# Gaukler/PlainRenderer

Hardware: AMD Instinct MI355X
Metric: frames/sec full GI+shade+post @4K; %HBM roofline; 1/2/4/8-GPU scaling (higher is better)
Workload: dtype f32

## Files before the change

### plainrenderer_amd/csrc/backend.cpp

```cpp
#include "backend.h"
#include "kernels_fast/pcf_taps.h"

#include <dlfcn.h>
#include <deque>
#include <algorithm>
#include <chrono>
#include <mutex>
#include <cstdlib>
#include <atomic>
#include <set>
#include <thread>
#include <unordered_map>
#include <unordered_set>
#include <cmath>
#include <cstring>
#include <map>
#include <memory>

#include "../../include/plr.h"

namespace plr {

struct ShaderEntry { std::string name; LaunchFn fn = nullptr; LaunchFn fast = nullptr; };
static bool shaderReadsBindless(const std::string& shader) {
// ... 211 lines not shown
    std::vector<FillOrder> fills;
    std::vector<uint8_t> fillData;
    static constexpr int kPinnedSlots = 3;
    struct PinnedSlot { void* host = nullptr; size_t size = 0; hipEvent_t free = nullptr; bool busy = false, eventPending = false; uint64_t serial = 0; } pinnedSlots[kPinnedSlots];
    uint64_t fillSerial = 0;
    uint32_t* edgeSignal = nullptr;
    uint32_t* edgeCounter = nullptr;
    uint32_t edgeSerial = 0;
    uint32_t pinnedNext = 0;
    uint32_t globalUbo = PLR_INVALID_INDEX;
    uint32_t layoutUbufs = 0, layoutSamplers = 0, layoutSampled = 0;
    bool layoutSet = false;
    ImgView* bindlessDev = nullptr;
    std::vector<ImgView> bindlessHost;
    uint32_t bindlessCapacity = 0;
    bool bindlessDirty = true;
    uint64_t allocated = 0;
    bool passTiming = false;
    int mathMode = PLR_MATH_FAST;
    std::vector<hipEvent_t> passEvents;
    struct Segment { size_t firstEvent; const char* name; };
    std::vector<Segment> segments;
    size_t eventsUsed = 0;
    const char* currentPassName = nullptr;
    bool timingNow = false;
    std::vector<plr_renderpass_time> lastTimings;
    std::set<std::string> callbackNames;
    size_t timedExecutions = 0;
    hipEvent_t frameStart = nullptr, frameEnd = nullptr;
    bool frameRecorded = false;
    bool frameTimeAsked = false;
    float lastFrameGpuMs = 0.f;
    float lastCpuMs = 0.f;
    static constexpr int kSideStreams = 3;
    hipStream_t sideStreams[kSideStreams] = {nullptr, nullptr, nullptr};
    std::vector<hipEvent_t> orderEvents;
    size_t orderEventsUsed = 0;
    bool overlap = false;
    int activeSideStreams = 1;
    hipStream_t curStream = nullptr;
    uint32_t lastOverlapped = 0;
    uint32_t* debugSig = nullptr;
    size_t debugSigWords = 0;
    int fusion = 2;
    GlobalUbo globalShadow{};
    bool globalShadowValid = false;
    uint32_t lastFused = 0;
    uint32_t lastGeneral = 0;
    std::string lastGeneralNames;
    uint64_t frameSerial = 0;
    hipStream_t tailStream = nullptr;
    hipEvent_t tailDone = nullptr, tailStart = nullptr;
    uint8_t* pendingFillSlot = nullptr;
    hipEvent_t pendingFillEvent = nullptr;

    hipStream_t earlyStream = nullptr;
    int earlyParts = 0;
    uint32_t lastEarly = 0;
    uint64_t mainOps = 0, tailStartOps = ~0ull;
    bool tailStartCoversLate = false, lateLaunchedThisFrame = false;
    std::vector<const void*> lastFillDsts;
    std::vector<EarlyPlan> earlyPlans;

    std::vector<Access> tailPending;
    bool asyncTail = true;
    bool fusionReorder = true;
    uint32_t lastAsync = 0;
    void* globalCopies[2] = {nullptr, nullptr};
    uint32_t globalCopyIndex = 0;
    std::set<std::string> fusedNames;
    std::unordered_map<const void*, uint64_t> contentVersion;
    std::unordered_set<const void*> externallyWritable;
};

static thread_local Backend* g = nullptr;
static thread_local std::string g_err;

static std::mutex g_exactSetMutex;
static bool g_exactSetTried = false;
static void* g_exactSetHandle = nullptr;
static std::string g_exactSetError;
static int ensureExactSet() {
    std::lock_guard<std::mutex> lock(g_exactSetMutex);
    if (!g_exactSetTried) {
        g_exactSetTried = true;
        Dl_info info{};
        std::string path;
        if (dladdr((const void*)&ensureExactSet, &info) && info.dli_fname) {
            path = info.dli_fname;
            const size_t slash = path.find_last_of('/');
            const size_t name = slash == std::string::npos ? 0 : slash + 1;
            if (path.compare(name, 6, "libplr") == 0) path.insert(name + 6, "_exact");
            else path.clear();
        }
        if (path.empty()) g_exactSetError = "cannot locate libplr.so to find libplr_exact.so next to it";
        else {
            g_exactSetHandle = dlopen(path.c_str(), RTLD_NOW | RTLD_LOCAL);
            if (!g_exactSetHandle) g_exactSetError = "the PLR_MATH_EXACT kernel set is a separate library and it did not load (" + path + "): " + (dlerror() ? dlerror() : "?") +
                                                     " - build it with plainrenderer_amd/build.py";
        }
    }
    if (!g_exactSetHandle) { g_err = g_exactSetError; return PLR_ERR_UNSUPPORTED; }
    return PLR_OK;
}

static std::string shaderBaseName(const std::string& path) {
// ... 222 lines not shown
        right = std::min(std::max(right, 0), (int)blocksX - left);
    }
    if (top + bottom > totalRows) return false;
    if (top + bottom + left + right == 0) return false;
    edgeTop = top; edgeBottom = bottom; total = totalRows;
    edgeLeft = left; edgeRight = right;
    edgeBlocks = (uint32_t)(top + bottom) * blocksX + (uint32_t)(left + right) * (uint32_t)(totalRows - top - bottom);
    edgeCounter = c.edgeCounter; edgeSignal = c.edgeSignal; edgeValue = c.edgeValue;
    if (edgeBlocks == 0) { edgeTop = edgeBottom = edgeLeft = edgeRight = 0; total = 0; return false; }
    static const bool orderOnly = std::getenv("PLR_EDGE_ORDER_ONLY") && std::atoi(std::getenv("PLR_EDGE_ORDER_ONLY")) != 0;
    if (orderOnly) { edgeBlocks = 0; return false; }
    c.edgeSignalHonoured = true;
    return true;
}

void countFusedExecutions(uint32_t n) { if (g) g->lastFused += n; }

}

using namespace plr;

extern "C" {

const char* plr_last_error(void) { return g_err.c_str(); }

int plr_setup(int device_ordinal, uint32_t width, uint32_t height) {
    if (g && g_adopted) { g = nullptr; g_adopted = false; }
    if (g) return setErr(PLR_ERR_INVALID_ARGUMENT, "plr_setup called twice; call plr_shutdown first");
    int count = 0;
    hipError_t e = hipGetDeviceCount(&count);
    if (e != hipSuccess || count == 0)
        return setErr(PLR_ERR_HIP, std::string("no HIP device available: ") + hipGetErrorString(e) + " (this backend has no CPU fallback)");
    if (device_ordinal < 0 || device_ordinal >= count) return setErr(PLR_ERR_INVALID_ARGUMENT, "device ordinal out of range");
    HIP_TRY(hipSetDevice(device_ordinal));
    g_ownedOnce = true;
    g = new Backend();
    {
        Backend* none = nullptr;
        g_first.compare_exchange_strong(none, g);
    }
    g->device = device_ordinal;
    int leastPriority = 0, greatestPriority = 0;
    if (hipDeviceGetStreamPriorityRange(&leastPriority, &greatestPriority) != hipSuccess) { (void)hipGetLastError(); leastPriority = greatestPriority = 0; }
    static const int mainPriority = std::getenv("PLR_MAIN_PRIORITY") ? std::atoi(std::getenv("PLR_MAIN_PRIORITY")) : 0;
    static const int earlyPriority = std::getenv("PLR_EARLY_PRIORITY") ? std::atoi(std::getenv("PLR_EARLY_PRIORITY")) : 0;
    if (mainPriority) HIP_TRY(hipStreamCreateWithPriority(&g->stream, hipStreamNonBlocking, greatestPriority));
    else HIP_TRY(hipStreamCreateWithFlags(&g->stream, hipStreamNonBlocking));
    HIP_TRY(hipEventCreate(&g->frameStart));
    HIP_TRY(hipEventCreate(&g->frameEnd));
    for (auto& slot : g->pinnedSlots) HIP_TRY(hipEventCreateWithFlags(&slot.free, hipEventDisableTiming));
    for (auto& st : g->sideStreams) HIP_TRY(hipStreamCreateWithFlags(&st, hipStreamNonBlocking));
    HIP_TRY(hipStreamCreateWithFlags(&g->tailStream, hipStreamNonBlocking));
    HIP_TRY(hipEventCreateWithFlags(&g->tailDone, hipEventDisableTiming));
    HIP_TRY(hipEventCreateWithFlags(&g->tailStart, hipEventDisableTiming));
    if (earlyPriority) HIP_TRY(hipStreamCreateWithPriority(&g->earlyStream, hipStreamNonBlocking, leastPriority));
    else HIP_TRY(hipStreamCreateWithFlags(&g->earlyStream, hipStreamNonBlocking));
    if (std::getenv("PLR_STREAM_DEBUG")) fprintf(stderr, "[plr streams] priority range least %d greatest %d; main %s, early %s\n", leastPriority, greatestPriority, mainPriority ? "greatest" : "default", earlyPriority ? "least" : "default");
    if (const char* ep = std::getenv("PLR_EARLY_PARTS")) g->earlyParts = std::min(std::max(std::atoi(ep), 0), 2);
    int canWaitValue = 0;
    if (hipDeviceGetAttribute(&canWaitValue, hipDeviceAttributeCanUseStreamWaitValue, device_ordinal) != hipSuccess) { (void)hipGetLastError(); canWaitValue = 0; }
    if (canWaitValue && hipExtMallocWithFlags((void**)&g->edgeSignal, 8, hipMallocSignalMemory) == hipSuccess && hipMalloc((void**)&g->edgeCounter, 4096) == hipSuccess) {
        HIP_TRY(hipMemset(g->edgeSignal, 0, 8));
        HIP_TRY(hipMemset(g->edgeCounter, 0, 4096));
    } else {
        (void)hipGetLastError();
        if (g->edgeSignal) hipFree(g->edgeSignal);
        g->edgeSignal = nullptr; g->edgeCounter = nullptr;
    }
    if (const char* es = std::getenv("PLR_EDGE_SIGNAL")) if (std::atoi(es) == 0 && g->edgeSignal) { hipFree(g->edgeSignal); hipFree(g->edgeCounter); g->edgeSignal = g->edgeCounter = nullptr; }
    if (const char* at = std::getenv("PLR_ASYNC_TAIL")) g->asyncTail = std::atoi(at) != 0;
    if (const char* ov = std::getenv("PLR_STREAM_OVERLAP")) g->overlap = std::atoi(ov) != 0;
    if (const char* pf = std::getenv("PLR_PASS_FUSION")) g->fusion = std::min(std::max(std::atoi(pf), 0), 2);
    if (const char* ns = std::getenv("PLR_SIDE_STREAMS")) g->activeSideStreams = std::min(std::max(std::atoi(ns), 1), (int)Backend::kSideStreams);
    return plr_recreate_swapchain(width, height);
}

int plr_shutdown(void) {
    if (!resolveBackend()) return PLR_OK;
    if (g_adopted) return setErr(PLR_ERR_INVALID_ARGUMENT, "plr_shutdown: this thread uses the backend another thread set up; that thread shuts it down");
    hipSetDevice(g->device);
    hipDeviceSynchronize();
    g->tailPending.clear();
    if (g->tailStream) hipStreamDestroy(g->tailStream);
    if (g->tailDone) hipEventDestroy(g->tailDone);
    if (g->tailStart) hipEventDestroy(g->tailStart);
    if (g->earlyStream) hipStreamDestroy(g->earlyStream);
    for (void* c : g->globalCopies) if (c) hipFree(c);
    if (g->edgeSignal) hipFree(g->edgeSignal);
    if (g->edgeCounter) hipFree(g->edgeCounter);
    for (auto& im : g->images) freeImage(im);
    for (auto& im : g->transient) freeImage(im);
    freeImage(g->swapchain);
    for (auto& b : g->ubufs) if (b.dev) hipFree(b.dev);
    for (auto& b : g->sbufs) if (b.dev) hipFree(b.dev);
    for (auto& p : g->passes) if (p->scratch.dev) hipFree(p->scratch.dev);
    if (g->debugSig) hipFree(g->debugSig);
    for (auto ev : g->passEvents) hipEventDestroy(ev);
    for (auto ev : g->orderEvents) hipEventDestroy(ev);
    for (auto st : g->sideStreams) if (st) hipStreamDestroy(st);
    if (g->bindlessDev) hipFree(g->bindlessDev);
    for (auto& slot : g->pinnedSlots) { if (slot.host) hipHostFree(slot.host); if (slot.free) hipEventDestroy(slot.free); }
    hipEventDestroy(g->frameStart); hipEventDestroy(g->frameEnd);
    hipStreamDestroy(g->stream);
    {
        Backend* mine = g;
        if (g_first.compare_exchange_strong(mine, nullptr)) g_firstEpoch++;
    }
// ... 296 lines not shown
            g->globalUbo = r->uniform_buffers[i].buffer;
        }
    }
    return PLR_OK;
}

static int fillPass(PassRes& p, const plr_compute_pass_desc* desc) {
    if (!desc || !desc->src_path_relative) return setErr(PLR_ERR_INVALID_ARGUMENT, "pass description / shader path is null");
    ShaderEntry found;
    const ShaderEntry* entry = findShader(desc->src_path_relative, &found) ? &found : nullptr;
    if (!entry) return setErr(PLR_ERR_UNKNOWN_SHADER, std::string("no HIP kernel for shader '") + desc->src_path_relative + "'");
    p.shader = desc->src_path_relative;
    if (desc->name) p.name = desc->name;
    p.fn = entry->fn;
    p.fast = entry->fast;
    p.readsBindless = shaderReadsBindless(entry->name);
    p.spec.clear();
    for (uint32_t i = 0; i < desc->specialisation_constant_count; i++) {
        const auto& s = desc->specialisation_constants[i];
        SpecConstant c;
        c.location = s.location;
        if (s.size) c.data.assign((const uint8_t*)s.data, (const uint8_t*)s.data + s.size);
        p.spec.push_back(std::move(c));
    }
    return PLR_OK;
}

int plr_update_compute_pass_shader_description(plr_pass_handle pass, const plr_compute_pass_desc* desc) {
    NEED_INIT();
    if (pass >= g->passes.size()) return setErr(PLR_ERR_INVALID_ARGUMENT, "invalid pass handle");
    plr_compute_pass_desc d = *desc;
    std::string keepName = g->passes[pass]->name;
    int rc = fillPass(*g->passes[pass], &d);
    if (!desc->name) g->passes[pass]->name = keepName;
    return rc;
}

int plr_create_compute_pass(const plr_compute_pass_desc* desc, plr_pass_handle* out_pass) {
    NEED_INIT();
    if (!out_pass) return setErr(PLR_ERR_INVALID_ARGUMENT, "out_pass is null");
    auto p = std::make_unique<PassRes>();
    int rc = fillPass(*p, desc);
    if (rc) return rc;
    g->passes.push_back(std::move(p));
    *out_pass = (plr_pass_handle)(g->passes.size() - 1);
    return PLR_OK;
}

constexpr uint32_t kFillKernelMaxBytes = 65536;
__global__ __launch_bounds__(256) void applyFillsKernel(uint8_t* __restrict__ slot, uint64_t serial) { applyFillsBlock(slot, serial); }

static int applyPendingFillsNow() {
    if (!g->pendingFillSlot) return PLR_OK;
    applyFillsKernel<<<1, 256, 0, g->stream>>>(g->pendingFillSlot, 0);
    HIP_TRY(hipGetLastError());
    g->mainOps++;
    g->pendingFillSlot = nullptr;
    if (g->pendingFillEvent) { HIP_TRY(hipEventRecord(g->pendingFillEvent, g->stream)); g->pendingFillEvent = nullptr; }
    return PLR_OK;
}

static int flushFills() {
    if (g->fills.empty()) return PLR_OK;
    if (int rc = applyPendingFillsNow()) return rc;
    const void* globalDev = g->globalUbo != PLR_INVALID_INDEX ? g->ubufs[g->globalUbo].dev : nullptr;
    bool globalFilled = false;
    for (const auto& f : g->fills) globalFilled = globalFilled || (globalDev && f.dst == globalDev);
    const bool copyGlobal = globalFilled && g->asyncTail;
    const size_t entryBytes = (g->fills.size() + 1) * sizeof(FillEntry);
    const size_t payloadBase = (kFillTableHeader + entryBytes + 15) & ~(size_t)15;
    const size_t need = payloadBase + g->fillData.size();
    Backend::PinnedSlot& slot = g->pinnedSlots[g->pinnedNext];
    g->pinnedNext = (g->pinnedNext + 1) % Backend::kPinnedSlots;
    if (slot.busy) {
        if (slot.eventPending) HIP_TRY(hipEventSynchronize(slot.free));
        else {
            volatile uint64_t* done = (volatile uint64_t*)((uint8_t*)slot.host + 8);
            for (uint32_t spins = 0; *done != slot.serial; spins++) {
                if (spins > 2000) { HIP_TRY(hipStreamSynchronize(g->stream)); break; }
                std::this_thread::yield();
            }
        }
        slot.busy = slot.eventPending = false;
    }
    if (slot.size < need) {
        if (slot.host) hipHostFree(slot.host);
        slot.size = std::max<size_t>(need * 2, 64 << 10);
        HIP_TRY(hipHostMalloc(&slot.host, slot.size, hipHostMallocDefault));
    }
    uint8_t* host = (uint8_t*)slot.host;
    std::memcpy(host + payloadBase, g->fillData.data(), g->fillData.size());
    for (const auto& f : g->fills)
        if (f.dst != globalDev && hazardWithTail({Access{f.dst, true}})) { if (int rc = joinAsyncTail()) return rc; break; }
    uint32_t count = 0;
    bool usedCopyEngine = false;
    FillEntry* entries = (FillEntry*)(host + kFillTableHeader);
    const FillOrder* lastGlobal = nullptr;
    for (const auto& f : g->fills) {
        if (f.size > kFillKernelMaxBytes || payloadBase + f.stagingOffset > 0xffffffffull) {
            if (count) {
                *(uint32_t*)host = count;
                applyFillsKernel<<<1, 256, 0, g->stream>>>(host, 0);
                HIP_TRY(hipGetLastError());
                HIP_TRY(hipStreamSynchronize(g->stream));
                count = 0;
            }
            HIP_TRY(hipMemcpyAsync(f.dst, host + payloadBase + f.stagingOffset, f.size, hipMemcpyHostToDevice, g->stream));
            g->mainOps++;
            usedCopyEngine = true;
        } else {
            entries[count++] = FillEntry{(uint64_t)(uintptr_t)f.dst, (uint32_t)(payloadBase + f.stagingOffset), (uint32_t)f.size};
        }
        if (globalDev && f.dst == globalDev) {
            std::memcpy(&g->globalShadow, (uint8_t*)slot.host + payloadBase + f.stagingOffset, std::min(f.size, sizeof(GlobalUbo)));
            if (f.size >= sizeof(GlobalUbo)) g->globalShadowValid = true;
            lastGlobal = &f;
        }
    }
    if (copyGlobal) {
        const uint32_t next = g->globalCopyIndex ^ 1u;
        if (!g->globalCopies[next]) HIP_TRY(hipMalloc(&g->globalCopies[next], sizeof(GlobalUbo)));
        if (hazardWithTail({Access{g->globalCopies[next], true}})) if (int rc = joinAsyncTail()) return rc;
        if (lastGlobal && lastGlobal->size >= sizeof(GlobalUbo) && lastGlobal->size <= kFillKernelMaxBytes) {
            entries[count++] = FillEntry{(uint64_t)(uintptr_t)g->globalCopies[next], (uint32_t)(payloadBase + lastGlobal->stagingOffset), (uint32_t)sizeof(GlobalUbo)};
        } else {
            if (count) { *(uint32_t*)host = count; applyFillsKernel<<<1, 256, 0, g->stream>>>(host, 0); HIP_TRY(hipGetLastError()); HIP_TRY(hipStreamSynchronize(g->stream)); count = 0; }
            HIP_TRY(hipMemcpyAsync(g->globalCopies[next], globalDev, sizeof(GlobalUbo), hipMemcpyDeviceToDevice, g->stream));
            g->mainOps++;
        }
        g->globalCopyIndex = next;
    }
    slot.serial = ++g->fillSerial;
    static const bool pollSlot = std::getenv("PLR_FILL_POLL") && std::atoi(std::getenv("PLR_FILL_POLL")) != 0;
    if (count && !usedCopyEngine && pollSlot) {
        *(uint32_t*)host = count;
        *(volatile uint64_t*)(host + 8) = 0;
        applyFillsKernel<<<1, 256, 0, g->stream>>>(host, slot.serial);
        HIP_TRY(hipGetLastError());
        g->mainOps++;
    } else {
        slot.eventPending = true;
        if (count && !usedCopyEngine) { *(uint32_t*)host = count; g->pendingFillSlot = host; g->pendingFillEvent = slot.free; }
        else {
            if (count) { *(uint32_t*)host = count; applyFillsKernel<<<1, 256, 0, g->stream>>>(host, 0); HIP_TRY(hipGetLastError()); }
            g->mainOps++;
            HIP_TRY(hipEventRecord(slot.free, g->stream));
        }
    }
    slot.busy = true;
    for (const auto& f : g->fills) g->lastFillDsts.push_back(f.dst);
    g->fills.clear();
    g->fillData.clear();
    return PLR_OK;
}

static int flushBindless() {
    if (!g->bindlessDirty) return PLR_OK;
    const uint32_t n = (uint32_t)g->images.size();
    if (n == 0) { g->bindlessHost.clear(); g->bindlessDirty = false; return PLR_OK; }
    if (g->bindlessCapacity < n) {
        HIP_TRY(hipStreamSynchronize(g->stream));
        if (g->bindlessDev) hipFree(g->bindlessDev);
        g->bindlessCapacity = std::max(n * 2, 64u);
        HIP_TRY(hipMalloc((void**)&g->bindlessDev, sizeof(ImgView) * g->bindlessCapacity));
    }
    std::vector<ImgView>& table = g->bindlessHost;
    table.resize(n);
    for (uint32_t i = 0; i < n; i++) {
        if (g->images[i].dev) table[i] = makeView(g->images[i], 0);
        else { table[i].ptr = nullptr; table[i].w = table[i].h = table[i].d = 0; table[i].fmt = -1; }
    }
    HIP_TRY(hipMemcpyAsync(g->bindlessDev, table.data(), sizeof(ImgView) * n, hipMemcpyHostToDevice, g->stream));
    HIP_TRY(hipStreamSynchronize(g->stream));
    g->bindlessDirty = false;
    return PLR_OK;
}

static int timingEvent(hipEvent_t* out) {
    if (g->eventsUsed == g->passEvents.size()) {
        hipEvent_t ev;
        HIP_TRY(hipEventCreate(&ev));
        g->passEvents.push_back(ev);
    }
    *out = g->passEvents[g->eventsUsed++];
    return PLR_OK;
}
static int beginSegment(const char* name) {
    hipEvent_t ev;
    if (int rc = timingEvent(&ev)) return rc;
    g->segments.push_back({g->eventsUsed - 1, name});
    HIP_TRY(hipEventRecord(ev, g->curStream ? g->curStream : g->stream));
    return PLR_OK;
}
static int endSegment() {
    hipEvent_t ev;
// ... 292 lines not shown
    return PLR_OK;
}

static int tryFusedLaunch(size_t i, size_t last, hipStream_t stream, const GlobalUbo* globalPtr, bool timed, size_t* covered) {
    *covered = 0;
    if (!g->fusion || g->mathMode != PLR_MATH_FAST) return PLR_OK;
    for (const FusionEntry& f : fusions()) {
        const size_t n = f.shaders.size();
        if (i + n > last) continue;
        if (g->debugSig && !f.writesSignatures) continue;
        bool match = true;
        for (size_t k = 0; k < n && match; k++) match = g->passes[g->executions[i + k].pass]->shader == f.shaders[k];
        for (size_t k = 0; k < n && match; k++) match = !g->executions[i + k].edgesFirst();
        if (!match) continue;
        const PassCtx* ctxs[8];
        if (n > 8) continue;
        for (size_t k = 0; k < n; k++) { prepareCtx(g->executions[i + k], stream, globalPtr); ctxs[k] = &g->executions[i + k].ctx; }
        EarlyPlan* early = nullptr;
        for (EarlyPlan& plan : g->earlyPlans) if (plan.launched && plan.group == i && plan.f == &f) early = &plan;
        if (early) {
            HIP_TRY(hipStreamWaitEvent(stream, early->done, 0));
            for (size_t k = 0; k < n; k++) g->executions[i + k].ctx.earlyPartDone = true;
        }
        if (g->fusion >= 2) {
            for (size_t k = 0; k < n; k++) {
                Execution& x = g->executions[i + k];
                for (int b = 0; b < kMaxBindings; b++) {
                    if (!x.ctx.hasStorage(b)) continue;
                    const void* key = nullptr;
                    for (const Access& a : x.access) if (a.write && a.key == x.ctx.storage[b].ptr) key = a.key;
                    if (!key) continue;
                    bool outside = false;
                    for (size_t j = 0; j < g->executions.size() && !outside; j++) {
                        if (j >= i && j < i + n) continue;
                        for (const Access& a : g->executions[j].access) if (a.key == key) { outside = true; break; }
                    }
                    if (!outside) x.ctx.elidableStorage |= 1u << b;
                }
            }
        }
        const char* label = nullptr;
        g->curStream = stream;
        if (timed) {
            std::string name;
            for (size_t k = 0; k < n; k++) name += (k ? " + " : "") + g->passes[g->executions[i + k].pass]->name;
            label = g->fusedNames.insert(name).first->c_str();
            if (int trc = beginSegment(label)) return trc;
        }
        g->currentPassName = label ? label : f.label.c_str();
        for (size_t k = 0; k < n; k++) touchAccesses(g->executions[i + k].access);
        Execution& first = g->executions[i];
        first.ctx.pendingFillSlot = nullptr; first.ctx.pendingFillsTaken = false; first.ctx.applyPendingFillsNow = nullptr;
        if (g->pendingFillSlot) {
            if (f.takesFills && stream == g->stream) { first.ctx.pendingFillSlot = g->pendingFillSlot; first.ctx.applyPendingFillsNow = &applyPendingFillsNow; }
            else if (int frc = applyPendingFillsNow()) return frc;
        }
        for (size_t k = 0; k < n; k++) if (int src = refuseStaleReads(g->executions[i + k], &g->executions[i], n)) return src;
        const int rc = f.fn(ctxs, n);
        if (first.ctx.pendingFillSlot) {
            if (rc == 0 && first.ctx.pendingFillsTaken) {
                g->pendingFillSlot = nullptr;
                if (g->pendingFillEvent) { HIP_TRY(hipEventRecord(g->pendingFillEvent, g->stream)); g->pendingFillEvent = nullptr; }
            } else if (rc == 0 && g->pendingFillSlot) { g_err = "fused launch '" + f.label + "' neither took nor applied the frame's pending fills"; return PLR_ERR_HIP; }
            first.ctx.pendingFillSlot = nullptr; first.ctx.applyPendingFillsNow = nullptr;
        }
        if (rc == kUseGeneralKernel) {
            if (early) { g_err = "fused launch '" + f.label + "' declined the bindings its early part accepted"; return PLR_ERR_HIP; }
            if (timed) { g->segments.pop_back(); g->eventsUsed -= 1; }
            continue;
        }
        if (rc) { g_err = "fused launch '" + f.label + "': " + g_err; return rc; }
        if (timed) if (int trc = endSegment()) return trc;
        for (size_t k = 0; k < n; k++) noteElidedImages(g->executions[i + k]);
        *covered = n;
        g->lastFused += (uint32_t)n;
        if (stream == g->stream) g->mainOps++;
        if (early) g->lateLaunchedThisFrame = true;
        return PLR_OK;
    }
    return PLR_OK;
}

static size_t fusionWindow(size_t i, size_t last) {
    size_t best = 1;
    if (!g->fusion || g->mathMode != PLR_MATH_FAST) return best;
    for (const FusionEntry& f : fusions()) {
        const size_t n = f.shaders.size();
        if (n <= best || i + n > last) continue;
        bool match = true;
        for (size_t k = 0; k < n && match; k++) match = g->passes[g->executions[i + k].pass]->shader == f.shaders[k];
        if (match) best = n;
    }
    return best;
}


static bool executionsConflict(const Execution& a, const Execution& b) {
    for (const Access& x : a.access)
        for (const Access& y : b.access) {
            if (x.key != y.key || !(x.write || y.write)) continue;
            if (x.key == kBindlessKey && x.write && y.write) continue;
            return true;
        }
    return false;
}
static void gatherFusionGroups() {
    if (!g->fusion || g->mathMode != PLR_MATH_FAST || g->overlap || g->debugSig) return;
// ... 629 lines not shown
```

### plainrenderer_amd/csrc/backend.h

```cpp
#pragma once
#include <hip/hip_runtime.h>
#include <stdint.h>
#include <cstring>
#include <memory>
#include <string>
#include <vector>

#include "device/image.h"
#include "device/types.h"

namespace plr {

constexpr int kMaxBindings = 32;

struct SpecConstant {
    uint32_t location;
    std::vector<uint8_t> data;
};

struct BufferBinding {
    void* ptr = nullptr;
    size_t size = 0;
    bool readOnly = false;
};

struct ScratchState { virtual ~ScratchState() = default; };
struct PassScratch { void* dev = nullptr; size_t bytes = 0; std::unique_ptr<ScratchState> state; };

struct PassCtx {
    hipStream_t stream = nullptr;
    const GlobalUbo* global = nullptr;
    const GlobalUbo* globalHost = nullptr;
    const ImgView* bindless = nullptr;
    const ImgView* bindlessHost = nullptr;
    uint32_t bindlessCount = 0;
    ImgView sampled[kMaxBindings];
    ImgView storage[kMaxBindings];
    uint32_t sampledMask = 0, storageMask = 0, sbufMask = 0, ubufMask = 0;
    BufferBinding sbuf[kMaxBindings];
    BufferBinding ubuf[kMaxBindings];
    std::vector<uint8_t> push;
    uint32_t dispatch[3] = {1, 1, 1};
    uint32_t base[3] = {0, 0, 0};
    uint32_t extraBaseY = 0, extraCountY = 0;
    uint8_t* pendingFillSlot = nullptr;
    mutable bool pendingFillsTaken = false;
    int (*applyPendingFillsNow)() = nullptr;
    uint32_t elidableStorage = 0;
    mutable uint32_t elidedStorage = 0;
    uint32_t firstRows[2] = {0, 0};
    uint32_t* edgeSignal = nullptr;
    uint32_t* edgeCounter = nullptr;
    uint32_t edgeValue = 0;
    mutable bool edgeSignalHonoured = false;
    uint32_t validRows[2] = {0, 0};
    uint32_t validCols[2] = {0, 0};
    uint32_t firstCols[2] = {0, 0};
    void validRowRange(int imageH, int* lo, int* hi) const {
        const bool all = validRows[0] == 0 && validRows[1] == 0;
        *lo = all ? 0 : (int)(validRows[0] < (uint32_t)imageH ? validRows[0] : (uint32_t)imageH);
        *hi = all ? imageH : (int)(validRows[1] < (uint32_t)imageH ? validRows[1] : (uint32_t)imageH);
    }
    void validColRange(int imageW, int* lo, int* hi) const {
        const bool all = validCols[0] == 0 && validCols[1] == 0;
        *lo = all ? 0 : (int)(validCols[0] < (uint32_t)imageW ? validCols[0] : (uint32_t)imageW);
        *hi = all ? imageW : (int)(validCols[1] < (uint32_t)imageW ? validCols[1] : (uint32_t)imageW);
    }
    const PassCtx* consumer = nullptr;
    mutable bool earlyPartDone = false;
    uint64_t frameSerial = 0;
    const std::vector<SpecConstant>* spec = nullptr;
    std::string* err = nullptr;
    PassScratch* passScratch = nullptr;
    uint32_t* debugSig = nullptr;
    size_t debugSigWords = 0;
    bool hostNoiseView(ImgView* out) const {
        if (!globalHost || !bindlessHost || bindlessCount == 0) return false;
        const uint32_t slot = (uint32_t)globalHost->noiseTextureIndices[globalHost->frameIndexMod4 & 3u];
        *out = bindlessHost[slot < bindlessCount - 1u ? slot : bindlessCount - 1u];
        return out->ptr != nullptr && out->w > 0 && out->h > 0;
    }
    uint32_t* sigFor(size_t pixels) const { return debugSig && debugSigWords >= pixels ? debugSig : nullptr; }

    bool hasSampled(int b) const { return (sampledMask >> b) & 1u; }
    bool hasStorage(int b) const { return (storageMask >> b) & 1u; }
    bool hasSbuf(int b) const { return (sbufMask >> b) & 1u; }
    bool hasUbuf(int b) const { return (ubufMask >> b) & 1u; }

    const SpecConstant* findSpec(uint32_t location) const;
    int32_t specInt(uint32_t location, int32_t def) const;
    uint32_t specUint(uint32_t location, uint32_t def) const { return (uint32_t)specInt(location, (int32_t)def); }
    float specFloat(uint32_t location, float def) const;
    bool specBool(uint32_t location, bool def) const;

    struct RowSpan { int y0, y1; };
    RowSpan rowSpan(int imageH, int wgRows = 8) const {
        const long long a = (long long)base[1] * wgRows, b = a + (long long)dispatch[1] * wgRows;
        RowSpan r;
// ... 167 lines not shown
```

### plainrenderer_amd/csrc/kernels_fast/histogram_fast.hip

```cpp
#include "../backend.h"
#include "../device/shading_common.h"
#include "../../../include/plr.h"
#include "fused_front.h"

namespace plr {

int launchHistogramThresholds(uint32_t* thresholds, uint32_t nBins, float minLuminance, float maxLuminance, hipStream_t stream);
int launchHistogramExactBins(uint8_t* out, uint32_t first, uint32_t count, uint32_t nBins, float minLuminance, float maxLuminance, hipStream_t stream);

namespace fasthist {

constexpr uint32_t kBins = 128;

PLR_DI uint32_t tableBin(float luminance, const float* thr, float guessScale, float guessBias) {
    const float g = __builtin_amdgcn_logf(luminance) * guessScale + guessBias;
    int gi = (int)__builtin_amdgcn_fmed3f(g, 0.f, (float)(kBins - 2u));
    const float lo = thr[gi], hi = thr[gi + 1];
    gi += (luminance >= hi) ? 1 : 0;
    gi -= (luminance >= lo) ? 0 : 1;
    return (uint32_t)max(gi, 0);
}

struct HistParams {
    ImgView src;
// ... 13 lines not shown
    const uint32_t* __restrict__ thresholds = p.thresholds;
    const float guessScale = p.guessScale, guessBias = p.guessBias;
    const uint32_t tilesX = p.tilesX;
    const uint32_t t = threadIdx.x;
    const uint32_t tileY = tileYIndex + p.tileY0;
    if (t < kBins) { localHistogram[t] = 0u; thr[t] = u2f(thresholds[t]); }
    __syncthreads();
    const int x0 = (int)tileXIndex * 32 + (int)(t & 7u) * 4;
    const int y = (int)tileY * 32 + (int)(t >> 3);
    const float prevExposure = light->previousFrameExposure;
    uint32_t texels[4] = {0u, 0u, 0u, 0u};
    int nValid = 0;
    if (y < src.h && x0 < src.w) {
        const uint32_t* row = (const uint32_t*)src.ptr + (size_t)y * (size_t)src.w;
        nValid = min(4, src.w - x0);
        if (nValid == 4 && ((src.w & 3) == 0)) {
            const uint4 v = *(const uint4*)(row + x0);
            texels[0] = v.x; texels[1] = v.y; texels[2] = v.z; texels[3] = v.w;
        } else {
            for (int i = 0; i < nValid; i++) texels[i] = row[x0 + i];
        }
    }
    uint32_t bins[4];
#pragma unroll
    for (int i = 0; i < 4; i++) {
        const vec3 c = unpackR11G11B10(texels[i]);
        const float luminance = dot(c, vec3(0.2126f, 0.7152f, 0.0722f)) / prevExposure;
        bins[i] = i < nValid ? tableBin(luminance, thr, guessScale, guessBias) : 0xffffffffu;
    }
#pragma unroll
    for (int i = 0; i < 4; i++) {
        if (bins[i] == 0xffffffffu) continue;
        uint32_t count = 1u;
#pragma unroll
        for (int j = i + 1; j < 4; j++)
            if (bins[j] == bins[i]) { count++; bins[j] = 0xffffffffu; }
        atomicAdd(&localHistogram[bins[i]], count);
    }
    __syncthreads();
    const uint32_t tileIndex = tileXIndex + tileY * tilesX;
    if (t < kBins) {
        const int rx = (int)tileXIndex * 32 + (int)(t & 31u), ry = (int)tileY * 32 + (int)(t >> 5);
        if (rx < src.w && ry < src.h) perTile[(size_t)tileIndex * kBins + t] = localHistogram[t];
    }
}

__global__ __launch_bounds__(256) void histogramPerTileFastKernel(HistParams p) {
    __shared__ uint32_t localHistogram[kBins];
    __shared__ float thr[kBins];
    histogramTileBlock(p, blockIdx.x, blockIdx.y, localHistogram, thr);
}

template <bool DOWNSCALE>
__global__ __launch_bounds__(256) void histogramAndPyramidKernel(HistParams p, fasthiz::QuadParams q, uint32_t histBlocks, uint32_t hizBlocks, uint32_t hizGridX, uint8_t* fillSlot) {
    __shared__ uint32_t localHistogram[kBins];
    __shared__ float thr[kBins];
    const uint32_t b = blockIdx.x;
    if (b == histBlocks + hizBlocks) { applyFillsBlock(fillSlot, 0); return; }
    const uint32_t paired = min(hizBlocks, histBlocks / 4u), remHist = histBlocks - 4u * paired;
    bool isHiz;
    uint32_t index;
    if (b < 5u * paired) { const uint32_t g = b / 5u, r = b % 5u; isHiz = r == 4u; index = isHiz ? g : 4u * g + r; }
    else { const uint32_t rem = b - 5u * paired; isHiz = rem >= remHist; index = isHiz ? paired + (rem - remHist) : 4u * paired + rem; }
    if (isHiz) fasthiz::hizQuadBlock<4, DOWNSCALE>(q, (int)(index % hizGridX) + q.tileX0, (int)(index / hizGridX) + q.tileY0);
    else histogramTileBlock(p, index % p.gridX, index / p.gridX, localHistogram, thr);
}

struct TableKey : ScratchState { float minL = 0.f, maxL = 0.f; bool valid = false; };

static int prepare(const PassCtx& c, HistParams* out) {
    if (!c.hasSampled(2) || c.sampled[2].fmt != F_R11G11B10 || !c.hasSbuf(3) || !c.hasSbuf(0)) return kUseGeneralKernel;
    const uint32_t nBins = c.specUint(0, 64u);
    const float minL = c.specFloat(1, 1.f), maxL = c.specFloat(2, 100.f);
    if (nBins != kBins || !(minL > 0.f) || !(maxL > minL)) return kUseGeneralKernel;
    const ImgView& src = c.sampled[2];
    const uint32_t tilesX = divUp((unsigned)src.w, 32u), tilesY = divUp((unsigned)src.h, 32u);
    if (c.sbuf[0].size < (size_t)tilesX * tilesY * nBins * 4u || c.sbuf[3].size < sizeof(LightBuffer)) return kUseGeneralKernel;
    const PassCtx::RowSpan rs = c.rowSpan((int)tilesY, 1);
    if (minL != 0.001f || maxL != 200000.f) return kUseGeneralKernel;
    uint32_t* thresholds = (uint32_t*)c.scratch(kBins * 4u);
    if (!thresholds) return c.fail(-2, "histogramPerTile: cannot allocate scratch memory");
    TableKey* key = c.scratchState<TableKey>();
    if (!key) return -1;
    if (!key->valid || key->minL != minL || key->maxL != maxL) {
        key->valid = false;
        if (launchHistogramThresholds(thresholds, kBins, minL, maxL, c.stream)) return c.fail(-2, "histogramPerTile: threshold table launch failed");
        key->minL = minL; key->maxL = maxL; key->valid = true;
    }
    const double logMin = std::log((double)minL), range = std::log((double)maxL) - logMin;
    out->src = src; out->light = (const LightBuffer*)c.sbuf[3].ptr; out->perTile = (uint32_t*)c.sbuf[0].ptr; out->thresholds = thresholds;
    out->guessScale = (float)(0.6931471805599453 / range * (kBins - 1u)); out->guessBias = (float)(-logMin / range * (kBins - 1u));
    const PassCtx::ColSpan cs = c.colSpan((int)tilesX, 1);
    out->tilesX = tilesX; out->tileY0 = (uint32_t)rs.y0; out->gridX = (uint32_t)(cs.x1 - cs.x0); out->gridY = rs.y1 > rs.y0 ? (uint32_t)(rs.y1 - rs.y0) : 0u;
    out->tileX0 = (uint32_t)cs.x0;
    return 0;
}
static int launch(const PassCtx& c) {
    HistParams p;
    if (int rc = prepare(c, &p)) return rc;
    if (p.gridY == 0 || p.gridX == 0) return 0;
    histogramPerTileFastKernel<<<dim3(p.gridX, p.gridY), 256, 0, c.stream>>>(p);
    PLR_CHECK_LAUNCH(c);
    return 0;
}

static int takeFillsIfDisjoint(const PassCtx& c, const HistParams& hp, uint8_t** fillSlot) {
    *fillSlot = nullptr;
    if (!c.pendingFillSlot) return 0;
    const uint8_t* slot = c.pendingFillSlot;
    const uint32_t nFills = *(const uint32_t*)slot;
    const FillEntry* entries = (const FillEntry*)(slot + kFillTableHeader);
    auto touches = [&](const void* base, size_t bytes) {
        for (uint32_t i = 0; i < nFills; i++)
            if (entries[i].dst < (uint64_t)(uintptr_t)base + bytes && (uint64_t)(uintptr_t)base < entries[i].dst + entries[i].size) return true;
        return false;
    };
    const bool disjoint = !touches(hp.light, sizeof(LightBuffer)) && !touches(hp.perTile, (size_t)hp.tilesX * (hp.tileY0 + hp.gridY) * kBins * 4u) &&
                          !touches(hp.thresholds, kBins * 4u);
    if (disjoint) { *fillSlot = c.pendingFillSlot; c.pendingFillsTaken = true; return 0; }
    return c.applyPendingFillsNow();
}

static int launchFusedFront(const PassCtx* const* ctxs, size_t count) {
    if (count != 6 && count != 8) return kUseGeneralKernel;
    HistParams hp;
    if (int rc = prepare(*ctxs[0], &hp)) return rc;
    if (hp.gridX == 0 || hp.gridY == 0 || hp.tileX0 != 0) return kUseGeneralKernel;
    ExposureChainPlan ep;
    if (int rc = prepareExposureChain(ctxs + 1, &ep)) return rc;
    if (ep.perTile != hp.perTile) return kUseGeneralKernel;
    fasthiz::Plan zp;
    if (int rc = fasthiz::prepare(*ctxs[4], ctxs[5], &zp)) return rc;
    FusedCullParams cull;
    int cullLevel = -1;
    if (zp.perTile) {
        if (count != 8) return kUseGeneralKernel;
        bool useHiZ = false;
        ImgView hiz;
        if (int rc = prepareFusedCulling(*ctxs[6], *ctxs[7], &cull, &useHiZ, &hiz)) return rc;
        const fasthiz::TileTailParams& t = zp.tileTail;
        if (!useHiZ || hiz.ptr != (const void*)t.level4 || hiz.w != t.w4 || hiz.h != t.h4) return kUseGeneralKernel;
        uint8_t* fillSlotT = nullptr;
        if (int rc = takeFillsIfDisjoint(*ctxs[0], hp, &fillSlotT)) return rc;
        const uint32_t histBlocksT = hp.gridX * hp.gridY, hizBlocksT = (uint32_t)(zp.gridX * zp.gridY);
        histogramAndPyramidKernel<true><<<histBlocksT + hizBlocksT + (fillSlotT ? 1u : 0u), 256, 0, ctxs[0]->stream>>>(hp, zp.quad, histBlocksT, hizBlocksT, (uint32_t)zp.gridX, fillSlotT);
        PLR_CHECK_LAUNCH(*ctxs[0]);
        return launchTileFrontSecondWithExposure(zp, cull, ep, ctxs[0]->stream);
    }
    if (count == 8) {
        bool useHiZ = false;
        ImgView hiz;
        if (int rc = prepareFusedCulling(*ctxs[6], *ctxs[7], &cull, &useHiZ, &hiz)) return rc;
        if (!useHiZ || zp.tailFirst < 1) return kUseGeneralKernel;
        for (int l = zp.tailFirst; l <= zp.tailFirst + 1 && l < zp.tail.count; l++)
            if (hiz.ptr == (const void*)zp.tail.level[l] && hiz.w == zp.tail.w[l] && hiz.h == zp.tail.h[l]) cullLevel = l;
        if (cullLevel < 0) return kUseGeneralKernel;
    }
    const uint32_t histBlocks = hp.gridX * hp.gridY, hizBlocks = (uint32_t)(zp.gridX * zp.gridY);
    uint8_t* fillSlot = nullptr;
    if (int rc = takeFillsIfDisjoint(*ctxs[0], hp, &fillSlot)) return rc;
    histogramAndPyramidKernel<true><<<histBlocks + hizBlocks + (fillSlot ? 1u : 0u), 256, 0, ctxs[0]->stream>>>(hp, zp.quad, histBlocks, hizBlocks, (uint32_t)zp.gridX, fillSlot);
    PLR_CHECK_LAUNCH(*ctxs[0]);
    return launchExposureChainAndPyramidTail(ep, zp, ctxs[0]->stream, count == 8 ? &cull : nullptr, cullLevel);
}

static int launchBandFront(const PassCtx* const* ctxs, size_t count) {
    if (count != 7) return kUseGeneralKernel;
    HistParams hp;
    if (int rc = prepare(*ctxs[0], &hp)) return rc;
    if (hp.gridX == 0 || hp.gridY == 0) return kUseGeneralKernel;
    ResetCombinePlan rp;
    if (int rc = prepareResetCombine(ctxs + 1, &rp)) return rc;
    if (rp.perTileBase != hp.perTile) return kUseGeneralKernel;
    fasthiz::Plan zp;
    if (int rc = fasthiz::prepare(*ctxs[3], ctxs[4], &zp)) return rc;
    if (!zp.perTile) return kUseGeneralKernel;
    FusedCullParams cull;
    bool useHiZ = false;
    ImgView hiz;
    if (int rc = prepareFusedCulling(*ctxs[5], *ctxs[6], &cull, &useHiZ, &hiz)) return rc;
    const fasthiz::TileTailParams& t = zp.tileTail;
    if (!useHiZ || hiz.ptr != (const void*)t.level4 || hiz.w != t.w4 || hiz.h != t.h4) return kUseGeneralKernel;
    uint8_t* fillSlot = nullptr;
    if (int rc = takeFillsIfDisjoint(*ctxs[0], hp, &fillSlot)) return rc;
    const uint32_t histBlocks = hp.gridX * hp.gridY, hizBlocks = (uint32_t)(zp.gridX * zp.gridY);
    histogramAndPyramidKernel<true><<<histBlocks + hizBlocks + (fillSlot ? 1u : 0u), 256, 0, ctxs[0]->stream>>>(hp, zp.quad, histBlocks, hizBlocks, (uint32_t)zp.gridX, fillSlot);
    PLR_CHECK_LAUNCH(*ctxs[0]);
    return launchBandFrontSecond(zp, cull, rp, ctxs[0]->stream);
}

__global__ void verifyKernel(const uint32_t* __restrict__ thresholds, const uint8_t* __restrict__ exact, uint32_t first, uint32_t count, float guessScale, float guessBias,
                             unsigned long long* __restrict__ mismatches) {
    __shared__ float thr[kBins];
    if (threadIdx.x < kBins) thr[threadIdx.x] = u2f(thresholds[threadIdx.x]);
    __syncthreads();
    const uint32_t i = blockIdx.x * blockDim.x + threadIdx.x;
    if (i >= count) return;
    if (tableBin(u2f(first + i), thr, guessScale, guessBias) != (uint32_t)exact[i]) atomicAdd(mismatches, 1ull);
}

}

static int fasthist_launch(const PassCtx& c) { return fasthist::launch(c); }
PLR_REGISTER_SHADER_FAST("histogramPerTile.comp", fasthist_launch);
static int fused_frame_front(const PassCtx* const* ctxs, size_t count) { return fasthist::launchFusedFront(ctxs, count); }
static int fused_band_front(const PassCtx* const* ctxs, size_t count) { return fasthist::launchBandFront(ctxs, count); }
PLR_REGISTER_FUSION_TAKES_FILLS("band front: histogram + reset + combine || per-tile depth pyramid || camera culling", fused_band_front, "histogramPerTile.comp", "histogramReset.comp", "histogramCombineTiles.comp",
                    "depthHiZPyramid.comp", "depthDownscale.comp", "sdfCameraFrustumCulling.comp", "sdfCameraTileCulling.comp");
static int fused_frame_front_and_culling(const PassCtx* const* ctxs, size_t count) { return fasthist::launchFusedFront(ctxs, count); }
PLR_REGISTER_FUSION_TAKES_FILLS("frame front: histogram + exposure chain || depth pyramid || camera culling", fused_frame_front_and_culling, "histogramPerTile.comp", "histogramReset.comp", "histogramCombineTiles.comp",
                    "preExposeLights.comp", "depthHiZPyramid.comp", "depthDownscale.comp", "sdfCameraFrustumCulling.comp", "sdfCameraTileCulling.comp");
PLR_REGISTER_FUSION_TAKES_FILLS("frame front: histogram + exposure chain || depth pyramid", fused_frame_front, "histogramPerTile.comp", "histogramReset.comp", "histogramCombineTiles.comp",
                    "preExposeLights.comp", "depthHiZPyramid.comp", "depthDownscale.comp");
}

using namespace plr;

extern "C" int plr_debug_verify_histogram_thresholds(float min_luminance, float max_luminance, uint64_t* out_mismatches) {
    if (!out_mismatches || !(min_luminance > 0.f) || !(max_luminance > min_luminance)) return setLastError(PLR_ERR_INVALID_ARGUMENT, "plr_debug_verify_histogram_thresholds: invalid argument");
    uint32_t* thresholds = nullptr;
    uint8_t* exact = nullptr;
    unsigned long long* counter = nullptr;
    const uint32_t chunk = 1u << 26;
    if (hipMalloc((void**)&thresholds, fasthist::kBins * 4u) != hipSuccess || hipMalloc((void**)&exact, chunk) != hipSuccess || hipMalloc((void**)&counter, 8) != hipSuccess)
        return setLastError(PLR_ERR_HIP, "plr_debug_verify_histogram_thresholds: hipMalloc failed");
    hipMemset(counter, 0, 8);
    int rc = launchHistogramThresholds(thresholds, fasthist::kBins, min_luminance, max_luminance, nullptr);
    const double logMin = std::log((double)min_luminance), range = std::log((double)max_luminance) - logMin;
    const float guessScale = (float)(0.6931471805599453 / range * (fasthist::kBins - 1u)), guessBias = (float)(-logMin / range * (fasthist::kBins - 1u));
    for (uint64_t first = 0; first < (1ull << 32) && !rc; first += chunk) {
        rc = launchHistogramExactBins(exact, (uint32_t)first, chunk, fasthist::kBins, min_luminance, max_luminance, nullptr);
        fasthist::verifyKernel<<<chunk / 256u, 256>>>(thresholds, exact, (uint32_t)first, chunk, guessScale, guessBias, counter);
    }
    unsigned long long host = ~0ull;
    const hipError_t e = hipMemcpy(&host, counter, 8, hipMemcpyDeviceToHost);
    hipFree(thresholds); hipFree(exact); hipFree(counter);
    if (rc || e != hipSuccess) return setLastError(PLR_ERR_HIP, "plr_debug_verify_histogram_thresholds: launch failed");
    *out_mismatches = host;
    return PLR_OK;
// ... 2 lines not shown
```

Before: 1481.

## Default to polled fill-slot completion and defer fills into fused kernels

```diff
diff --git a/plainrenderer_amd/csrc/backend.cpp b/plainrenderer_amd/csrc/backend.cpp
--- a/plainrenderer_amd/csrc/backend.cpp
+++ b/plainrenderer_amd/csrc/backend.cpp
@@ -287,6 +287,8 @@
     hipStream_t tailStream = nullptr;
     hipEvent_t tailDone = nullptr, tailStart = nullptr;
     uint8_t* pendingFillSlot = nullptr;
+    bool fillPoll = true;
+    uint64_t pendingFillSerial = 0;
     hipEvent_t pendingFillEvent = nullptr;
 
     hipStream_t earlyStream = nullptr;
@@ -615,7 +617,9 @@
     for (auto& st : g->sideStreams) HIP_TRY(hipStreamCreateWithFlags(&st, hipStreamNonBlocking));
     HIP_TRY(hipStreamCreateWithFlags(&g->tailStream, hipStreamNonBlocking));
     HIP_TRY(hipEventCreateWithFlags(&g->tailDone, hipEventDisableTiming));
-    HIP_TRY(hipEventCreateWithFlags(&g->tailStart, hipEventDisableTiming));
+    g->fillPoll = !(std::getenv("PLR_FILL_POLL") && std::atoi(std::getenv("PLR_FILL_POLL")) == 0);
+    const bool tailStartFence = std::getenv("PLR_TAIL_START_FENCE") && std::atoi(std::getenv("PLR_TAIL_START_FENCE")) != 0;
+    HIP_TRY(hipEventCreateWithFlags(&g->tailStart, hipEventDisableTiming | (tailStartFence ? 0u : (unsigned)hipEventDisableSystemFence)));
     if (earlyPriority) HIP_TRY(hipStreamCreateWithPriority(&g->earlyStream, hipStreamNonBlocking, leastPriority));
     else HIP_TRY(hipStreamCreateWithFlags(&g->earlyStream, hipStreamNonBlocking));
     if (std::getenv("PLR_STREAM_DEBUG")) fprintf(stderr, "[plr streams] priority range least %d greatest %d; main %s, early %s\n", leastPriority, greatestPriority, mainPriority ? "greatest" : "default", earlyPriority ? "least" : "default");
@@ -1018,7 +1022,7 @@
 
 static int applyPendingFillsNow() {
     if (!g->pendingFillSlot) return PLR_OK;
-    applyFillsKernel<<<1, 256, 0, g->stream>>>(g->pendingFillSlot, 0);
+    applyFillsKernel<<<1, 256, 0, g->stream>>>(g->pendingFillSlot, g->pendingFillSerial);
     HIP_TRY(hipGetLastError());
     g->mainOps++;
     g->pendingFillSlot = nullptr;
@@ -1042,8 +1046,9 @@
         if (slot.eventPending) HIP_TRY(hipEventSynchronize(slot.free));
         else {
             volatile uint64_t* done = (volatile uint64_t*)((uint8_t*)slot.host + 8);
+            const auto giveUp = std::chrono::steady_clock::now() + std::chrono::milliseconds(250);
             for (uint32_t spins = 0; *done != slot.serial; spins++) {
-                if (spins > 2000) { HIP_TRY(hipStreamSynchronize(g->stream)); break; }
+                if ((spins & 1023u) == 1023u && std::chrono::steady_clock::now() > giveUp) { HIP_TRY(hipStreamSynchronize(g->stream)); break; }
                 std::this_thread::yield();
             }
         }
@@ -1097,16 +1102,13 @@
         g->globalCopyIndex = next;
     }
     slot.serial = ++g->fillSerial;
-    static const bool pollSlot = std::getenv("PLR_FILL_POLL") && std::atoi(std::getenv("PLR_FILL_POLL")) != 0;
-    if (count && !usedCopyEngine && pollSlot) {
+    if (count && !usedCopyEngine && g->fillPoll) {
         *(uint32_t*)host = count;
         *(volatile uint64_t*)(host + 8) = 0;
-        applyFillsKernel<<<1, 256, 0, g->stream>>>(host, slot.serial);
-        HIP_TRY(hipGetLastError());
-        g->mainOps++;
+        g->pendingFillSlot = host; g->pendingFillSerial = slot.serial; g->pendingFillEvent = nullptr;
     } else {
         slot.eventPending = true;
-        if (count && !usedCopyEngine) { *(uint32_t*)host = count; g->pendingFillSlot = host; g->pendingFillEvent = slot.free; }
+        if (count && !usedCopyEngine) { *(uint32_t*)host = count; g->pendingFillSlot = host; g->pendingFillSerial = 0; g->pendingFillEvent = slot.free; }
         else {
             if (count) { *(uint32_t*)host = count; applyFillsKernel<<<1, 256, 0, g->stream>>>(host, 0); HIP_TRY(hipGetLastError()); }
             g->mainOps++;
@@ -1505,7 +1507,7 @@
         Execution& first = g->executions[i];
         first.ctx.pendingFillSlot = nullptr; first.ctx.pendingFillsTaken = false; first.ctx.applyPendingFillsNow = nullptr;
         if (g->pendingFillSlot) {
-            if (f.takesFills && stream == g->stream) { first.ctx.pendingFillSlot = g->pendingFillSlot; first.ctx.applyPendingFillsNow = &applyPendingFillsNow; }
+            if (f.takesFills && stream == g->stream) { first.ctx.pendingFillSlot = g->pendingFillSlot; first.ctx.pendingFillSerial = g->pendingFillSerial; first.ctx.applyPendingFillsNow = &applyPendingFillsNow; }
             else if (int frc = applyPendingFillsNow()) return frc;
         }
         for (size_t k = 0; k < n; k++) if (int src = refuseStaleReads(g->executions[i + k], &g->executions[i], n)) return src;
diff --git a/plainrenderer_amd/csrc/backend.h b/plainrenderer_amd/csrc/backend.h
--- a/plainrenderer_amd/csrc/backend.h
+++ b/plainrenderer_amd/csrc/backend.h
@@ -44,6 +44,7 @@
     uint32_t base[3] = {0, 0, 0};
     uint32_t extraBaseY = 0, extraCountY = 0;
     uint8_t* pendingFillSlot = nullptr;
+    uint64_t pendingFillSerial = 0;
     mutable bool pendingFillsTaken = false;
     int (*applyPendingFillsNow)() = nullptr;
     uint32_t elidableStorage = 0;
diff --git a/plainrenderer_amd/csrc/kernels_fast/histogram_fast.hip b/plainrenderer_amd/csrc/kernels_fast/histogram_fast.hip
--- a/plainrenderer_amd/csrc/kernels_fast/histogram_fast.hip
+++ b/plainrenderer_amd/csrc/kernels_fast/histogram_fast.hip
@@ -89,11 +89,11 @@
 }
 
 template <bool DOWNSCALE>
-__global__ __launch_bounds__(256) void histogramAndPyramidKernel(HistParams p, fasthiz::QuadParams q, uint32_t histBlocks, uint32_t hizBlocks, uint32_t hizGridX, uint8_t* fillSlot) {
+__global__ __launch_bounds__(256) void histogramAndPyramidKernel(HistParams p, fasthiz::QuadParams q, uint32_t histBlocks, uint32_t hizBlocks, uint32_t hizGridX, uint8_t* fillSlot, uint64_t fillSerial) {
     __shared__ uint32_t localHistogram[kBins];
     __shared__ float thr[kBins];
     const uint32_t b = blockIdx.x;
-    if (b == histBlocks + hizBlocks) { applyFillsBlock(fillSlot, 0); return; }
+    if (b == histBlocks + hizBlocks) { applyFillsBlock(fillSlot, fillSerial); return; }
     const uint32_t paired = min(hizBlocks, histBlocks / 4u), remHist = histBlocks - 4u * paired;
     bool isHiz;
     uint32_t index;
@@ -180,7 +180,7 @@
         uint8_t* fillSlotT = nullptr;
         if (int rc = takeFillsIfDisjoint(*ctxs[0], hp, &fillSlotT)) return rc;
         const uint32_t histBlocksT = hp.gridX * hp.gridY, hizBlocksT = (uint32_t)(zp.gridX * zp.gridY);
-        histogramAndPyramidKernel<true><<<histBlocksT + hizBlocksT + (fillSlotT ? 1u : 0u), 256, 0, ctxs[0]->stream>>>(hp, zp.quad, histBlocksT, hizBlocksT, (uint32_t)zp.gridX, fillSlotT);
+        histogramAndPyramidKernel<true><<<histBlocksT + hizBlocksT + (fillSlotT ? 1u : 0u), 256, 0, ctxs[0]->stream>>>(hp, zp.quad, histBlocksT, hizBlocksT, (uint32_t)zp.gridX, fillSlotT, ctxs[0]->pendingFillSerial);
         PLR_CHECK_LAUNCH(*ctxs[0]);
         return launchTileFrontSecondWithExposure(zp, cull, ep, ctxs[0]->stream);
     }
@@ -196,7 +196,7 @@
     const uint32_t histBlocks = hp.gridX * hp.gridY, hizBlocks = (uint32_t)(zp.gridX * zp.gridY);
     uint8_t* fillSlot = nullptr;
     if (int rc = takeFillsIfDisjoint(*ctxs[0], hp, &fillSlot)) return rc;
-    histogramAndPyramidKernel<true><<<histBlocks + hizBlocks + (fillSlot ? 1u : 0u), 256, 0, ctxs[0]->stream>>>(hp, zp.quad, histBlocks, hizBlocks, (uint32_t)zp.gridX, fillSlot);
+    histogramAndPyramidKernel<true><<<histBlocks + hizBlocks + (fillSlot ? 1u : 0u), 256, 0, ctxs[0]->stream>>>(hp, zp.quad, histBlocks, hizBlocks, (uint32_t)zp.gridX, fillSlot, ctxs[0]->pendingFillSerial);
     PLR_CHECK_LAUNCH(*ctxs[0]);
     return launchExposureChainAndPyramidTail(ep, zp, ctxs[0]->stream, count == 8 ? &cull : nullptr, cullLevel);
 }
@@ -221,7 +221,7 @@
     uint8_t* fillSlot = nullptr;
     if (int rc = takeFillsIfDisjoint(*ctxs[0], hp, &fillSlot)) return rc;
     const uint32_t histBlocks = hp.gridX * hp.gridY, hizBlocks = (uint32_t)(zp.gridX * zp.gridY);
-    histogramAndPyramidKernel<true><<<histBlocks + hizBlocks + (fillSlot ? 1u : 0u), 256, 0, ctxs[0]->stream>>>(hp, zp.quad, histBlocks, hizBlocks, (uint32_t)zp.gridX, fillSlot);
+    histogramAndPyramidKernel<true><<<histBlocks + hizBlocks + (fillSlot ? 1u : 0u), 256, 0, ctxs[0]->stream>>>(hp, zp.quad, histBlocks, hizBlocks, (uint32_t)zp.gridX, fillSlot, ctxs[0]->pendingFillSerial);
     PLR_CHECK_LAUNCH(*ctxs[0]);
     return launchBandFrontSecond(zp, cull, rp, ctxs[0]->stream);
 }
```

Result: no change. 1496, median of 6 (+1.0%).
